# joekurina/Agilex-NTT

Measured on AMD Instinct MI355X. Metric: batched n=4096 forward NTTs/sec at 1/2/4/8 MI355X; %HBM roofline, higher is better.
Workload: dtype u64; 1 GPU; n=4096, 4-prime RNS (60-bit), batch=4096 polynomials per GPU, forward negacyclic NTT in place (BASELINE.json configs[2]); n=4096, primes=4, batch_per_gpu=4096, slabs_rotated=4, clock_ramp_steps_before_warmup=1856, parallelism=batch-sharded x1, no collective

## Files before the change

agilex-ntt_amd/csrc/agx_ntt.cpp:

```cpp
#include "../../include/agx_ntt.h"

#include <hip/hip_runtime.h>

#include <algorithm>
#include <cmath>
#include <cstdlib>
#include <cstring>
#include <memory>
#include <mutex>
#include <new>
#include <vector>

#include "host_math.hpp"
#include "operands.hpp"
#include "plan_internal.hpp"
#include "rb_registry.hpp"
#ifdef AGX_DIAG
#include "../../tools/agx_ntt_diag.h"
#endif

using namespace agx;

thread_local int g_last_hip_error = 0;

// ... 72 lines not shown

int check_modulus(uint64_t q, uint32_t n) {
    if (q < 3 || (q & 1) == 0 || q >= (1ull << 62)) return AGX_ERR_BAD_MODULUS;
    if ((q - 1) % (2ull * n)) return AGX_ERR_BAD_MODULUS;
    return AGX_OK;
}

int check_shape(uint32_t n, uint32_t num_primes) {
    if (int rc = check_size(n)) return rc;
    return num_primes == 0 || num_primes > 65535 ? AGX_ERR_BAD_ARGUMENT : AGX_OK;
}

int check_create_args(uint32_t n, uint32_t num_primes, const uint64_t* moduli, const uint64_t* tw, const uint64_t* pre, const uint64_t* itw, const uint64_t* ipre) {
    if (!moduli || !tw || !pre || (itw == nullptr) != (ipre == nullptr)) return AGX_ERR_NULL_POINTER;
    if (int rc = check_shape(n, num_primes)) return rc;
    for (uint32_t k = 0; k < num_primes; ++k)
        if (int rc = check_modulus(moduli[k], n)) return rc;
    return AGX_OK;
}

int check_plan(const agx_ntt_plan* plan) {
    if (!plan) return AGX_ERR_NULL_POINTER;
    int dev = -1;
    return hipGetDevice(&dev) == hipSuccess && dev == plan->device ? AGX_OK : AGX_ERR_BAD_ARGUMENT;
}

void free_plan(agx_ntt_plan* p) {
    if (!p) return;
    for (hipEvent_t ev : p->ticket_events)
        if (ev) (void)hipEventDestroy(ev);
    delete p;
}

static std::vector<ulonglong2> build_pass_table(const rb_entry* e, const std::vector<ulonglong2>& pairs, uint32_t num_primes, uint32_t n) {
    std::vector<ulonglong2> out;
    std::vector<uint64_t> w(n), wp(n);
    for (uint32_t k = 0; k < num_primes; ++k) {
        for (uint32_t j = 0; j < n; ++j) w[j] = pairs[(size_t)k * n + j].x, wp[j] = pairs[(size_t)k * n + j].y;
        e->build(w.data(), wp.data(), out);
    }
    return out;
}

static void resolve_routes(agx_ntt_plan* p) {
    route generic;
    generic.n = p->n, generic.log_n = p->log_n, generic.num_primes = p->num_primes;
    generic.consts = p->d_consts, generic.tw = p->d_tw, generic.itw = p->d_itw, generic.rescale = p->d_rescale;
    generic.ticket_for = &plan_ticket_for, generic.ticket_launched = &plan_ticket_launched;
    generic.ticket_ctx = p;
    auto through = [&](const pass_tables& t) {
        route r = generic;
        r.rb = t.entry, r.tw_rb = t.fwd, r.itw_rb = t.inv;
        return r;
    };
    const rb_entry* e = p->variant == AGX_VARIANT_LDS_RADIX2 ? nullptr : p->main.entry;
    const route main = e ? through(p->main) : generic;
    const bool inv = e && p->main.inv;
    plan_routes& r = p->routes;
    r.forward = main;
    const bool large = e && !p->explicit_id && p->chosen.forward_large && p->chosen.forward_large == p->companion.entry;
    r.forward_large = large ? through(p->companion) : route{};
    r.min_frames = p->chosen.min_frames;
    r.inverse = inv && e->launch_inv ? main : generic;
    r.polymul = inv && e->launch_mul ? main : generic;
    r.polymul_ntt = inv && e->launch_mulhat ? main : generic;
    r.rescale = inv && e->launch_rescale ? main : generic;
    r.extend = e && e->launch_extend ? main : generic;
    r.moddown = inv && e->launch_moddown ? main : generic;
}

static const route& forward_route(const agx_ntt_plan* p, uint64_t batch) {
    const plan_routes& r = p->routes;
// ... 48 lines not shown
        c.mu_lo = (uint64_t)mu;
        if (q >= (1ull << 58) && q <= (1ull << 60)) {
            float f = (float)(4294967296.0 / (double)q * (1.0 - 1.0 / 1048576.0));
            if ((double)f > 4294967296.0 / (double)q * (1.0 - 1.0 / 1048576.0)) f = std::nextafterf(f, 0.0f);
            uint32_t bits;
            std::memcpy(&bits, &f, sizeof(bits));
            c.est = bits;
        }
        c.est |= (uint64_t)q60c_of(q) << 32;

        c.n_inv = inv_pow2_mod(img.log_n, q);
        c.n_inv_p = shoup_quotient(c.n_inv, q);
        const uint64_t* twk = tw + (size_t)k * n;
        const uint64_t* prek = pre + (size_t)k * n;
        for (uint32_t j = 0; j < n; ++j) img.tw_pairs[(size_t)k * n + j] = make_ulonglong2(twk[j], prek[j]);
        if (itw) {
            const uint64_t* itwk = itw + (size_t)k * n;
            const uint64_t* iprek = ipre + (size_t)k * n;
            for (uint32_t j = 0; j < n; ++j) img.itw_pairs[(size_t)k * n + j] = make_ulonglong2(itwk[j], iprek[j]);
            c.w1n = mul_mod(itwk[1] % q, c.n_inv, q);
            c.w1n_p = shoup_quotient(c.w1n, q);
        }
    }
    img.rescale_legal = num_primes >= 2;
    img.rescale.assign(num_primes >= 2 ? num_primes - 1 : 0, rescale_consts{});
    for (uint32_t k = 0; k + 1 < num_primes; ++k) {
        const uint64_t q = moduli[k], q_last = moduli[num_primes - 1], h = (q_last - 1) >> 1;
        rescale_consts& rc = img.rescale[k];
        rc.q_last = q_last, rc.h = h, rc.h_mod_q = h % q;
        if (inv_mod_euclid(q_last, q, &rc.qlinv)) rc.qlinv_p = shoup_quotient(rc.qlinv, q);
        else img.rescale_legal = false;
    }
    const rb_selection& c = img.chosen;
    if (c.main) img.tables.push_back({c.main, build_pass_table(c.main, img.tw_pairs, num_primes, n), itw ? build_pass_table(c.main, img.itw_pairs, num_primes, n) : std::vector<ulonglong2>{}});
    if (c.forward_large && c.forward_large != c.main) img.tables.push_back({c.forward_large, build_pass_table(c.forward_large, img.tw_pairs, num_primes, n), {}});
}

static int upload_pass_tables(pass_tables& dst, const host_pass_tables& src) {
    dst.entry = src.entry;
    if (int rc = dst.fwd.upload(src.fwd)) return rc;
    return src.inv.empty() ? AGX_OK : dst.inv.upload(src.inv);
}

int prepare_auto_image(plan_image& img, uint32_t n, uint32_t num_primes, const uint64_t* moduli, const uint64_t* psi) {
    std::vector<uint64_t> roots(num_primes), tw((size_t)num_primes * n), pre(tw.size()), itw(tw.size()), ipre(tw.size());
    for (uint32_t k = 0; k < num_primes; ++k) {
        const uint64_t q = moduli[k];
        if (int rc = check_modulus(q, n)) return rc;
        if (!is_prime_u64(q)) return AGX_ERR_BAD_MODULUS;
        roots[k] = psi ? psi[k] : min_primitive_root_2n(q, n);
        if (!is_primitive_root_2n(roots[k], q, n)) return AGX_ERR_BAD_ROOT;
        power_tables_bitrev(q, roots[k], n, &tw[(size_t)k * n], &pre[(size_t)k * n]);
        power_tables_bitrev(q, inv_mod(roots[k], q), n, &itw[(size_t)k * n], &ipre[(size_t)k * n]);
    }
    prepare_plan_image(img, n, num_primes, moduli, roots.data(), tw.data(), pre.data(), itw.data(), ipre.data());
    return AGX_OK;
}

int instantiate_plan(agx_ntt_plan** out, const plan_image& img) {
    int ndev = 0;
    if (hipGetDeviceCount(&ndev) != hipSuccess || ndev == 0) return AGX_ERR_NO_DEVICE;
    std::unique_ptr<agx_ntt_plan, void (*)(agx_ntt_plan*)> p(new (std::nothrow) agx_ntt_plan, &free_plan);
    if (!p) return AGX_ERR_ALLOC;
    p->n = img.n, p->log_n = img.log_n, p->num_primes = img.num_primes;
    p->has_inverse = img.has_inverse, p->arith_level = img.arith_level, p->narrow_level = img.narrow_level;
    p->chosen = img.chosen;
    p->rescale_legal = img.rescale_legal;
    p->ticket_streams.reserve(kTicketSlots);
// ... 37 lines not shown
int check_frames(const agx_ntt_plan* plan, const void* base, const frame_layout& fl) {
    if (!base) return AGX_ERR_NULL_POINTER;
    if (!aligned8(base) || !batch_fits_grid(plan, fl.batch)) return AGX_ERR_BAD_ARGUMENT;
    if (fl.batch > 1 && fl.poly_stride < (int64_t)plan->n) return AGX_ERR_BAD_ARGUMENT;
    if (!layout_fits(plan->n, plan->num_primes, fl.batch, fl.prime_stride, fl.poly_stride)) return AGX_ERR_BAD_ARGUMENT;
    if (self_overlap(plan->n, plan->num_primes, fl.batch, fl.prime_stride, fl.poly_stride)) return AGX_ERR_BAD_ARGUMENT;
    return AGX_OK;
}

int check_pair(const agx_ntt_plan* plan, const void* base, const void* other, const frame_layout& fl) {
    if (!other) return AGX_ERR_NULL_POINTER;
    if (!aligned8(other)) return AGX_ERR_BAD_ARGUMENT;
    return partial_overlap(addr(base), addr(other), plan->n, plan->num_primes, fl.batch, fl.prime_stride, fl.poly_stride) ? AGX_ERR_BAD_ARGUMENT : AGX_OK;
}

static int plan_set_variant_impl(agx_ntt_plan* plan, int variant) {
    if (!plan) return AGX_ERR_NULL_POINTER;
    int config_id = -1;
    if (variant >= AGX_VARIANT_REGBLOCK_BASE) {
        config_id = variant - AGX_VARIANT_REGBLOCK_BASE;
        variant = AGX_VARIANT_REGBLOCK;
    }
    if (variant != AGX_VARIANT_AUTO && variant != AGX_VARIANT_LDS_RADIX2 && variant != AGX_VARIANT_REGBLOCK) return AGX_ERR_BAD_ARGUMENT;
    if (variant != AGX_VARIANT_LDS_RADIX2) {
        rb_selection sel = regblock_select(plan->n, config_id, plan->arith_level, plan->narrow_level);
        if (!sel.main) {
            if (variant == AGX_VARIANT_REGBLOCK) return AGX_ERR_BAD_SIZE;
            sel.main = plan->main.entry;
        }
        if (sel.main != plan->main.entry) {
            host_pass_tables host{sel.main, {}, {}};
            std::vector<ulonglong2> pairs((size_t)plan->num_primes * plan->n);
            AGX_HIP(hipMemcpy(pairs.data(), plan->d_tw, pairs.size() * sizeof(ulonglong2), hipMemcpyDeviceToHost));
            host.fwd = build_pass_table(sel.main, pairs, plan->num_primes, plan->n);
            if (plan->d_itw) {
                AGX_HIP(hipMemcpy(pairs.data(), plan->d_itw, pairs.size() * sizeof(ulonglong2), hipMemcpyDeviceToHost));
                host.inv = build_pass_table(sel.main, pairs, plan->num_primes, plan->n);
            }
            pass_tables fresh;
            if (int rc = upload_pass_tables(fresh, host)) return rc;
            AGX_HIP(hipDeviceSynchronize());
            plan->main = std::move(fresh);
        }
        plan->chosen = sel;
        plan->explicit_id = config_id >= 0;
    }
    plan->variant = variant;
    resolve_routes(plan);
    return AGX_OK;
}

}

extern "C" {

const char* agx_ntt_strerror(int status) {
    switch (status) {
        case AGX_OK: return "success";
        case AGX_ERR_NULL_POINTER: return "required pointer argument is NULL";
        case AGX_ERR_BAD_SIZE: return "n must be a power of two in [2, 32768]";
        case AGX_ERR_BAD_MODULUS: return "modulus must be an odd prime < 2^62 with q = 1 (mod 2n)";
        case AGX_ERR_BAD_ROOT: return "psi is not a primitive 2n-th root of unity mod q";
        case AGX_ERR_BAD_ARGUMENT: return "invalid argument";
        case AGX_ERR_NO_DEVICE: return "no HIP device available";
        case AGX_ERR_HIP: return "HIP runtime error (see agx_ntt_last_hip_error)";
        case AGX_ERR_ALLOC: return "allocation failed";
        case AGX_ERR_NO_INVERSE: return "plan has no inverse tables";
    }
    return "unknown status";
}
// ... 503 lines not shown
```

agilex-ntt_amd/csrc/host_math.cpp:

```cpp
#include "host_math.hpp"

namespace agx {

typedef unsigned __int128 u128;

uint64_t mul_mod(uint64_t a, uint64_t b, uint64_t q) { return (uint64_t)((u128)a * b % q); }

uint64_t pow_mod(uint64_t a, uint64_t e, uint64_t q) {
    uint64_t r = 1 % q, base = a % q;
    for (; e; e >>= 1) {
        if (e & 1) r = mul_mod(r, base, q);
        base = mul_mod(base, base, q);
    }
    return r;
}

uint64_t inv_mod(uint64_t a, uint64_t q) { return pow_mod(a, q - 2, q); }

bool is_prime_u64(uint64_t q) {
    if (q < 2) return false;
    const uint64_t wit[] = {2, 3, 5, 7, 11, 13, 17, 19, 23, 29, 31, 37};
    for (uint64_t p : wit)
        if (q % p == 0) return q == p;
    uint64_t odd = q - 1;
// ... 32 lines not shown

uint64_t min_primitive_root_2n(uint64_t q, uint32_t n) {
    const uint64_t two_n = 2ull * n;
    if (q < 3 || (q - 1) % two_n) return 0;
    const uint64_t cofactor = (q - 1) / two_n;
    uint64_t some_root = 0;
    for (uint64_t g = 2; g < q && g < 100000; ++g) {
        uint64_t r = pow_mod(g, cofactor, q);
        if (is_primitive_root_2n(r, q, n)) { some_root = r; break; }
    }
    if (!some_root) return 0;
    const uint64_t sq = mul_mod(some_root, some_root, q);
    uint64_t least = some_root, walk = some_root;
    for (uint32_t k = 1; k < n; ++k) {
        walk = mul_mod(walk, sq, q);
        if (walk < least) least = walk;
    }
    return least;
}

bool inv_mod_euclid(uint64_t a, uint64_t q, uint64_t* inv) {
    __int128 r0 = q, r1 = a % q, t0 = 0, t1 = 1;
    while (r1 != 0) {
        const __int128 k = r0 / r1, r2 = r0 - k * r1, t2 = t0 - k * t1;
        r0 = r1, r1 = r2, t0 = t1, t1 = t2;
    }
    if (r0 != 1) return false;
    *inv = (uint64_t)(t0 < 0 ? t0 + (__int128)q : t0);
    return true;
}

uint64_t shoup_quotient(uint64_t w, uint64_t q) { return (uint64_t)(((u128)w << 64) / q); }

void power_tables_bitrev(uint64_t q, uint64_t base, uint32_t n, uint64_t* tw, uint64_t* pre) {
    const int lg = log2u(n);
    std::vector<uint64_t> pw(n);
    pw[0] = 1 % q;
    for (uint32_t i = 1; i < n; ++i) pw[i] = mul_mod(pw[i - 1], base, q);
    for (uint32_t j = 0; j < n; ++j) {
        tw[j] = pw[bit_reverse(j, lg)];
        pre[j] = shoup_quotient(tw[j], q);
    }
}

bool basis_constants(const uint64_t* src, uint32_t S, const uint64_t* dst, uint32_t T, uint64_t* dinv, uint64_t* dinv_p, uint64_t* mat, uint64_t* mat_p) {
    auto d_mod = [&](uint32_t i, uint64_t m) {
        uint64_t r = 1 % m;
        for (uint32_t k = 0; k < S; ++k)
            if (k != i) r = mul_mod(r, src[k] % m, m);
        return r;
    };
    for (uint32_t i = 0; i < S; ++i) {
        if (!inv_mod_euclid(d_mod(i, src[i]), src[i], &dinv[i])) return false;
        dinv_p[i] = shoup_quotient(dinv[i], src[i]);
    }
    for (uint32_t j = 0; j < T; ++j)
        for (uint32_t i = 0; i < S; ++i) {
            mat[(std::size_t)j * S + i] = d_mod(i, dst[j]);
            mat_p[(std::size_t)j * S + i] = shoup_quotient(mat[(std::size_t)j * S + i], dst[j]);
        }
    return true;
}

bool moddown_constants(const uint64_t* src, uint32_t S, const uint64_t* dst, uint32_t T, const uint64_t* dinv, const uint64_t* n_inv, const uint64_t* w1n,
                       uint64_t* dall, uint64_t* dall_p, uint64_t* sn, uint64_t* sn_p, uint64_t* sw, uint64_t* sw_p) {
    for (uint32_t i = 0; i < S; ++i) {
// ... 18 lines not shown
```

agilex-ntt_amd/csrc/host_math.hpp:

```cpp
#pragma once
#include <cstddef>
#include <cstdint>
#include <vector>

namespace agx {

uint64_t mul_mod(uint64_t a, uint64_t b, uint64_t q);
uint64_t pow_mod(uint64_t a, uint64_t e, uint64_t q);
uint64_t inv_mod(uint64_t a, uint64_t q);
bool inv_mod_euclid(uint64_t a, uint64_t q, uint64_t* inv);
bool is_prime_u64(uint64_t q);
inline bool is_pow2(uint32_t n) { return n && !(n & (n - 1)); }
inline int log2u(uint32_t n) { int l = 0; while ((1u << l) < n) ++l; return l; }
inline uint32_t bit_reverse(uint32_t x, int bits) {
    uint32_t r = 0;
    for (int i = 0; i < bits; ++i) { r = (r << 1) | (x & 1u); x >>= 1; }
    return r;
}

std::vector<uint64_t> find_ntt_primes(uint32_t bits, uint32_t n, uint32_t count);
uint64_t min_primitive_root_2n(uint64_t q, uint32_t n);
bool is_primitive_root_2n(uint64_t psi, uint64_t q, uint32_t n);

uint64_t shoup_quotient(uint64_t w, uint64_t q);
void power_tables_bitrev(uint64_t q, uint64_t base, uint32_t n, uint64_t* tw, uint64_t* pre);

bool basis_constants(const uint64_t* src, uint32_t S, const uint64_t* dst, uint32_t T, uint64_t* dinv, uint64_t* dinv_p, uint64_t* mat, uint64_t* mat_p);

bool moddown_constants(const uint64_t* src, uint32_t S, const uint64_t* dst, uint32_t T, const uint64_t* dinv, const uint64_t* n_inv, const uint64_t* w1n,
                       uint64_t* dall, uint64_t* dall_p, uint64_t* sn, uint64_t* sn_p, uint64_t* sw, uint64_t* sw_p);

}
```

agilex-ntt_amd/csrc/modarith.hpp:

```cpp
#pragma once
#include <hip/hip_runtime.h>
#include <cstdint>

namespace agx {

typedef ulonglong2 twpair;

__device__ __forceinline__ uint64_t mul_shoup_lazy(uint64_t y, uint64_t w, uint64_t wp, uint64_t q) {
    const uint64_t c = __umul64hi(y, wp);
    return w * y - c * q;
}

__device__ __forceinline__ uint64_t csub(uint64_t v, uint64_t m) { return v >= m ? v - m : v; }

__device__ __forceinline__ uint64_t reduce_4q(uint64_t v, uint64_t q, uint64_t q2) {
    return csub(csub(v, q2), q);
}

__device__ __forceinline__ void ct_butterfly(uint64_t& x, uint64_t& y, uint64_t w, uint64_t wp,
                                             uint64_t q, uint64_t q2) {
    const uint64_t tx = csub(x, q2);
    const uint64_t qv = mul_shoup_lazy(y, w, wp, q);
    x = tx + qv;
    y = tx + q2 - qv;
// ... 43 lines not shown
}


__device__ __forceinline__ uint64_t mad64(uint32_t a, uint32_t b, uint64_t c) { return (uint64_t)a * b + c; }
__device__ __forceinline__ uint64_t mul64(uint32_t a, uint32_t b) { return (uint64_t)a * b; }

template <int TAG>
__device__ __forceinline__ uint32_t opaque_one() {
    uint32_t one;
    if constexpr (TAG == 0) asm("s_mov_b32 %0, 1" : "=s"(one));
    else asm("s_movk_i32 %0, 0x1" : "=s"(one));
    return one;
}
__device__ __forceinline__ uint64_t add64_32(uint64_t c, uint32_t a, uint32_t one) { return (uint64_t)a * one + c; }

__device__ __forceinline__ uint64_t opaque_sgpr64(uint64_t v) {
    asm("" : "+s"(v));
    return v;
}

__device__ __forceinline__ uint64_t keep64(uint64_t v) {
    asm("" : "+v"(v));
    return v;
}

struct bf_consts {
    uint64_t q;
    uint64_t nq;
    uint64_t m;
    uint64_t nm;
    uint32_t one_a, one_b;
    float est_inv;
    uint32_t c, c8;
};

__device__ __forceinline__ uint64_t csub_sign(uint64_t x, const bf_consts& k) {
    const uint64_t d = x + k.nm;
    const uint32_t neg = (uint32_t)((int32_t)(uint32_t)(d >> 32) >> 31);
    typedef uint32_t u32x2 __attribute__((ext_vector_type(2)));
    u32x2 add;
    add.x = neg & (uint32_t)k.m;
    add.y = neg & (uint32_t)(k.m >> 32);
    return d + __builtin_bit_cast(uint64_t, add);
}

template <int VAR = 0>
__device__ __forceinline__ uint64_t fold_product(uint64_t tx, uint64_t y, uint64_t w, uint64_t c, const bf_consts& k) {
    const uint32_t y0 = (uint32_t)y, y1 = (uint32_t)(y >> 32), w0 = (uint32_t)w, w1 = (uint32_t)(w >> 32);
    const uint32_t c0 = (uint32_t)c, c1 = (uint32_t)(c >> 32), nq0 = (uint32_t)k.nq, nq1 = (uint32_t)(k.nq >> 32);
    uint64_t acc = mad64(w0, y0, tx);
    acc = mad64(nq0, c0, acc);
    if constexpr (VAR == 1) {
        const uint32_t z32 = w0 * y1 + w1 * y0 + nq1 * c0 + nq0 * c1;
        typedef uint32_t u32x2v __attribute__((ext_vector_type(2)));
        u32x2v av = __builtin_bit_cast(u32x2v, acc);
        av.y += z32;
        return __builtin_bit_cast(uint64_t, av);
    }
    uint64_t z = mul64(w0, y1);
    z = mad64(w1, y0, z);
    z = mad64(nq1, c0, z);
    z = keep64(mad64(nq0, c1, z));
    typedef uint32_t u32x2 __attribute__((ext_vector_type(2)));
    u32x2 a = __builtin_bit_cast(u32x2, acc);
    a.y += (uint32_t)z;
    return __builtin_bit_cast(uint64_t, a);
// ... 176 lines not shown
        return lazy16_tailfree::valid(total);
    }
};

__device__ __forceinline__ uint64_t csub_8q_q60c(uint64_t x, const bf_consts& k) {
    typedef uint32_t u32x2 __attribute__((ext_vector_type(2)));
    u32x2 v = __builtin_bit_cast(u32x2, x);
    uint32_t s = v.y >> 31;
    asm("" : "+v"(s));
    v.y &= 0x7fffffffu;
    return mad64(s, k.c8, __builtin_bit_cast(uint64_t, v));
}

template <bool DO_CSUB>
__device__ __forceinline__ void ct_butterfly_q60c(uint64_t& x, uint64_t& y, uint64_t w, uint64_t wp, const bf_consts& k) {
    const uint32_t y0 = (uint32_t)y, y1 = (uint32_t)(y >> 32), p0 = (uint32_t)wp, p1 = (uint32_t)(wp >> 32);
    const uint64_t tx = DO_CSUB ? csub_8q_q60c(x, k) : x;
    uint64_t c = mad64(p1, y1, (uint64_t)__umulhi(y0, p1));
    c = add64_32(c, __umulhi(y1, p0), k.one_b);
    const uint64_t xn = fold_product(tx, y, w, c, k);
    y = (tx << 1) + k.m - xn;
    x = xn;
}

__device__ __forceinline__ uint64_t reduce_final_q60c(uint64_t v, const bf_consts& k, const final_consts& f, bool lazy_out) {
    typedef uint32_t u32x2 __attribute__((ext_vector_type(2)));
    u32x2 r = __builtin_bit_cast(u32x2, v);
    const uint32_t kq = r.y >> 28;
    r.y &= 0x0fffffffu;
    const uint64_t t = mad64(kq, k.c, __builtin_bit_cast(uint64_t, r));
    return lazy_out ? t : csub_select_c(t, f.nq1);
}

template <bool FAST>
__device__ __forceinline__ uint64_t mul_shoup_form(uint64_t d, uint64_t w, uint64_t wp, const bf_consts& k) {
    const uint32_t d0 = (uint32_t)d, d1 = (uint32_t)(d >> 32), p0 = (uint32_t)wp, p1 = (uint32_t)(wp >> 32);
    uint64_t c;
    if constexpr (FAST) {
        c = mad64(p1, d1, (uint64_t)__umulhi(d0, p1));
        c = add64_32(c, __umulhi(d1, p0), k.one_b);
    } else {
        const uint32_t t = __umulhi(d0, p0);
        const uint64_t m1 = add64_32(mul64(p1, d0), t, k.one_a);
        const uint64_t m2 = add64_32(mul64(p0, d1), (uint32_t)m1, k.one_b);
        c = add64_32(mul64(p1, d1), (uint32_t)(m1 >> 32), k.one_a);
        c = add64_32(c, (uint32_t)(m2 >> 32), k.one_b);
    }
    return fold_product(0, d, w, c, k);
}

template <bool FAST, bool SEL = false>
__device__ __forceinline__ void gs_butterfly_form(uint64_t& x, uint64_t& y, uint64_t w, uint64_t wp, const bf_consts& k) {
    const uint64_t s = x + y;
    const uint64_t d = x + k.m - y;
    if constexpr (FAST) x = SEL ? csub_select(s, k) : csub_sign(s, k);
    else x = csub(s, k.m);
    y = mul_shoup_form<FAST>(d, w, wp, k);
}

template <bool FAST>
__device__ __forceinline__ void gs_last_form(uint64_t& x, uint64_t& y, uint64_t ninv, uint64_t ninv_p,
                                             uint64_t w1n, uint64_t w1n_p, const bf_consts& k) {
    const uint64_t s = x + y;
    const uint64_t d = x + k.m - y;
    x = mul_shoup_form<FAST>(s, ninv, ninv_p, k);
    y = mul_shoup_form<FAST>(d, w1n, w1n_p, k);
// ... 52 lines not shown
```

agilex-ntt_amd/csrc/rb32_kernels.hpp:

```cpp
#pragma once

namespace agx {
namespace AGX_TU {

typedef uint2 tw32;
typedef unsigned long long u64x2 __attribute__((ext_vector_type(2)));

__device__ __forceinline__ tw32 load_uniform32(const tw32* p) {
    typedef const uint64_t __attribute__((address_space(4))) * const_ptr;
    const uint64_t v = *(const_ptr)(uintptr_t)p;
    return make_uint2((uint32_t)v, (uint32_t)(v >> 32));
}

__device__ __forceinline__ uint32_t csub32(uint32_t a, uint32_t m) {
    const uint32_t d = a - m;
    return d < a ? d : a;
}

template <int TIER>
struct q32_arith {
    static_assert(TIER == 1 || TIER == 2, "1: q < 2^31, 2: q < 2^30");
    uint32_t q, q2;
    __device__ __forceinline__ void init(uint64_t q64) {
        q = (uint32_t)q64;
// ... 260 lines not shown
polymul_q32(const uint64_t* __restrict__ pa, const uint64_t* __restrict__ pb, uint64_t* __restrict__ pcout, const prime_consts* __restrict__ consts,
            const twpair* __restrict__ tw_rb, const twpair* __restrict__ itw_rb, uint32_t pairs_per_prime, uint64_t frames_x,
            int64_t prime_stride, int64_t poly_stride, uint32_t flags) {
    __builtin_amdgcn_s_setprio(3);
    AGX_RB32_PROLOGUE;
    (void)wide;
    const tw32* itbl = reinterpret_cast<const tw32*>(itw_rb) + (size_t)prime * pairs_per_prime * 2;
    uint32_t xa[C], xb[C];
    {
        uint64_t va[C];
        static_for<0, C>([&](auto Rr) { constexpr int r = Rr; va[r] = __builtin_nontemporal_load(&pa[base + f.tid + (uint32_t)r * T]); });
        asm volatile("" ::: "memory");
        __builtin_amdgcn_s_setprio(0);
        static_for<0, C>([&](auto Rr) { constexpr int r = Rr; xa[r] = f.a.template enter<false>(va[r]); });
    }
    f.forward(xa, tbl, true);
    asm volatile("" ::: "memory");
    static_for<0, C>([&](auto Rr) { constexpr int r = Rr; xb[r] = f.a.template enter<false>(__builtin_nontemporal_load(&pb[base + f.tid + (uint32_t)r * T])); });
    __syncthreads();
    {
        const tw32* tbl2 = tbl;
        asm volatile("" : "+s"(tbl2));
        f.forward(xb, tbl2, true);
    }
    static_for<0, C>([&](auto Rr) { constexpr int r = Rr; xa[r] = f.a.mulmod(xa[r], xb[r], pc.mu_hi); });
    const tw32 ninv = make_uint2((uint32_t)pc.n_inv, (uint32_t)(pc.n_inv_p >> 32)), w1n = make_uint2((uint32_t)pc.w1n, (uint32_t)(pc.w1n_p >> 32));
    f.inverse(xa, itbl, ninv, w1n);
    if (live) {
        static_for<0, C>([&](auto Rr) { constexpr int r = Rr; __builtin_nontemporal_store((uint64_t)xa[r], &pcout[base + f.tid + (uint32_t)r * T]); });
    }
}

template <int L, int R>
void build_table32_t(const uint64_t* tw, const uint64_t* pre, std::vector<ulonglong2>& out) {
    using G = rb_geom<L, R>;
    static_assert(G::table_pairs % 2 == 0, "two 8-byte entries per 16-byte slot");
    std::vector<uint2> t((size_t)G::table_pairs, make_uint2(0, 0));
    for_each_table_slot<L, R>([&](size_t at, uint32_t idx) { t[at] = make_uint2((uint32_t)tw[idx], (uint32_t)(pre[idx] >> 32)); });
    const size_t start = out.size();
    out.resize(start + (size_t)G::table_pairs / 2);
    std::memcpy(out.data() + start, t.data(), t.size() * sizeof(uint2));
}

template <int L, int R, int PPB, int TIER, int MINW>
struct q32_shape {
    static constexpr int log_n = L, r = R, fpb = PPB, threads = rb_geom<L, R>::T * PPB, min_waves = MINW, arith = 1, narrow = TIER;
    static constexpr uint32_t table_pairs = rb_geom<L, R>::table_pairs / 2;
    static constexpr size_t lds = (size_t)((1u << L) + (1u << (L - 5))) * 4 * PPB;
    static constexpr auto build = &build_table32_t<L, R>;
    static constexpr bool flags_everywhere = true;
    static uint32_t flags(const void* a, const void* b, const void* c, const frame_layout& fl) {
        const bool aligned = (((uintptr_t)a | (uintptr_t)b | (uintptr_t)c) & 15u) == 0 && ((fl.prime_stride | fl.poly_stride) & 1) == 0;
        return (fl.lazy_out ? 1u : 0u) | (aligned ? 2u : 0u);
    }
};

template <int L, int R, int PPB, int TIER, int MINW>
constexpr rb_entry make_entry_q32(int id) {
    return make_entry3<q32_shape<L, R, PPB, TIER, MINW>, &fwd_q32<L, R, PPB, TIER, MINW>, &inv_q32<L, R, PPB, TIER, MINW>, &polymul_q32<L, R, PPB, TIER, MINW>>(id);
}

}
}
```

agilex-ntt_amd/csrc/rb_frame.hpp:

```cpp
#pragma once
#include "rb_registry.hpp"
#include "modarith.hpp"

#include <algorithm>
#include <cstdlib>
#include <type_traits>
#include <utility>

#ifndef AGX_POLYMUL_MAXW
#define AGX_POLYMUL_MAXW 5
#endif
#ifndef AGX_TU
#error "define AGX_TU (a per-translation-unit namespace name) before including rb_frame.hpp / rb_kernels.hpp"
#endif

namespace agx {
namespace AGX_TU {



template <int B, int E, typename F>
__device__ __host__ __forceinline__ void static_for(F&& f) {
    if constexpr (B < E) {
        f(std::integral_constant<int, B>{});
// ... 60 lines not shown
    return {r0, r0 | (1 << rb), b >> rb};
}

struct no_op {
    __device__ __forceinline__ void operator()() const {}
};
template <int C, class WR, class RD, class SYNC, class MID = no_op>
__device__ __forceinline__ void split_words_out(const uint64_t (&x)[C], uint32_t* w, uint32_t (&lo)[C], WR&& wr, RD&& rd, SYNC&& sync, MID&& mid = MID{}) {
    static_for<0, C>([&](auto r) { w[wr(r)] = (uint32_t)x[r]; });
    mid();
    sync();
    static_for<0, C>([&](auto r) { lo[r] = w[rd(r)]; });
    sync();
    static_for<0, C>([&](auto r) { w[wr(r)] = (uint32_t)(x[r] >> 32); });
    sync();
}

constexpr int kOptPad = 1;
constexpr int kOptSelect = 2;
constexpr int kOptLazy16 = 16;
constexpr int kOptTwAhead = 32;
constexpr int kOptTrace = 64;
constexpr int kOptPrio = 128;
constexpr int kOptPrioBarrier = 512;
constexpr int kOptScalarBase = 1024;
constexpr int kOptLazyInv = 2048;
constexpr int kOptTwAheadInv = 4096;
constexpr int kOptNtLoad = 131072, kOptNtStore = 262144;
constexpr int kOptEstReduce = 524288;
constexpr int kOptSplitWord = 1048576;
constexpr int kOptStreamTw = 1 << 25;
constexpr int kOptPinBf = 1 << 26;
constexpr int kOptQ60c = 1 << 27;
constexpr int kOptStreamCh1 = 1 << 29;

#ifdef AGX_DIAG
__device__ uint64_t* g_trace_buf = nullptr;
__device__ uint64_t g_trace_waves = 0;
#endif

template <int L, int R, bool FAST, int OPT = 0>
struct rb2_frame {
    using G = rb2_geom<L, R>;
    static constexpr int C = G::C, T = G::T, NP = G::NP;
    static constexpr bool FAST_ARITH = FAST, SEL = (OPT & kOptSelect) != 0, LAZY16 = FAST && (OPT & kOptLazy16) != 0;
    static_assert((OPT & kOptPad) != 0, "every kernel uses the padded image");
    static constexpr bool TWA = (OPT & kOptTwAhead) != 0 && R >= 3;
    static constexpr bool TRACE = (OPT & kOptTrace) != 0;
    static constexpr bool PRIO = (OPT & kOptPrio) != 0;
    static constexpr bool PRIO_BARRIER = PRIO && (OPT & kOptPrioBarrier) != 0, SCALAR_BASE = (OPT & kOptScalarBase) != 0;
    static constexpr bool LAZY_INV = LAZY16 && (OPT & kOptLazyInv) != 0;
    static constexpr bool NT_LOAD = (OPT & kOptNtLoad) != 0, NT_STORE = (OPT & kOptNtStore) != 0;
    static constexpr bool TWA_INV = (OPT & kOptTwAheadInv) != 0 && R == 3;
    static constexpr bool EST = LAZY16 && SEL && (OPT & kOptEstReduce) != 0;
    static constexpr bool Q60C = EST && (OPT & kOptQ60c) != 0;
    static constexpr bool SPLIT = (OPT & kOptSplitWord) != 0;
    static constexpr bool STREAM_TW = (OPT & kOptStreamTw) != 0, PIN_BF = (OPT & kOptPinBf) != 0, STREAM_CH1 = (OPT & kOptStreamCh1) != 0;
    static_assert(!EST || lazy16_tailfree::valid(L), "tail-free schedule must keep every stage within 16q");
    static_assert(!Q60C || q60c_tailfree::valid(L), "sign-bit subtracts must keep every stage within 16q + 8c");
    mutable uint64_t ts[12];
    uint64_t trace_wave = ~0ull;
    bool trace_wait_stores = true;
    template <int I>
    __device__ __forceinline__ void stamp(uint64_t& anchor) const {
        if constexpr (TRACE) {
            uint64_t t;
            asm volatile("s_memtime %0\n\ts_waitcnt lgkmcnt(0)" : "=s"(t), "+v"(anchor) : : "memory");
            ts[I] = t;
        }
    }
    __device__ __forceinline__ void trace_flush() const {
#ifndef AGX_DIAG
        static_assert(!TRACE, "kOptTrace kernels belong to the diagnostics library (AGX_DIAG): the product library has no trace buffer");
#else
        if constexpr (TRACE) {
            const uint64_t wave = ((uint64_t)blockIdx.y * gridDim.x + blockIdx.x) * (blockDim.x >> 6) + (threadIdx.x >> 6);
            if ((threadIdx.x & 63u) == 0 && g_trace_buf != nullptr && wave < g_trace_waves) {
                uint64_t* dst = g_trace_buf + wave * 16;
#pragma unroll
                for (int i = 0; i < 12; ++i) dst[i] = ts[i];
                dst[12] = __builtin_amdgcn_s_getreg((31 << 11) | 4);
                dst[13] = __builtin_amdgcn_s_getreg((31 << 11) | 20);
            }
        }
#endif
    }
    static constexpr bool lane_full_pass(int p) { return p >= 0 && p < NP && G::rlo(p) < 6 && G::hi(p) - G::rlo(p) + 1 == R; }
    static constexpr int PADS = SPLIT ? 5 : 4;
    static constexpr uint32_t slab_elems = (1u << L) + (L >= PADS ? (1u << (L >= PADS ? L - PADS : 0)) : 0u);
    static constexpr uint32_t image_bytes = slab_elems * (SPLIT ? 4u : 8u);
    static __device__ __forceinline__ constexpr uint32_t img(uint32_t e) { return e + (e >> PADS); }
    uint32_t tid;
    bool lazy_out = false;
    uint64_t* slab;
    bf_consts k;
    final_consts fc;

    __device__ __forceinline__ void init_consts(uint64_t q, uint64_t est = 0) {
        k.est_inv = __uint_as_float((uint32_t)est);
        k.q = q;
        k.nq = 0 - q;
        k.m = FAST ? (q << 2) : (q << 1);
        k.nm = opaque_sgpr64(0 - k.m);
        k.one_a = opaque_one<0>();
        k.one_b = opaque_one<1>();
        fc.q2 = q << 1;
        fc.nq2 = opaque_sgpr64(0 - fc.q2);
        fc.q1 = q;
        fc.nq1 = opaque_sgpr64(0 - fc.q1);
        fc.q8 = q << 3;
        fc.nq8 = opaque_sgpr64(0 - fc.q8);
        if constexpr (Q60C) {
            k.c = (uint32_t)(est >> 32);
            k.c8 = k.c << 3;
        }
    }

    template <int stage>
    __device__ __forceinline__ void butterfly(uint64_t& a, uint64_t& b, const twpair& w) const {
        if constexpr (Q60C) ct_butterfly_q60c<lazy16_tailfree::subtracts(stage, L)>(a, b, w.x, w.y, k);
        else if constexpr (EST) ct_butterfly_lazy16<SEL, lazy16_tailfree::subtracts(stage, L), false>(a, b, w.x, w.y, k, fc);
        else if constexpr (LAZY16) ct_butterfly_lazy16<SEL, lazy16_schedule::subtracts(stage), stage == L - 1>(a, b, w.x, w.y, k, fc);
        else if constexpr (FAST) ct_butterfly_fast<SEL>(a, b, w.x, w.y, k);
        else ct_butterfly_exact(a, b, w.x, w.y, k);
    }

    template <int stage, int MODE>
    __device__ __forceinline__ void forward_step(uint64_t& a, uint64_t& b, const twpair& w) const {
        butterfly<stage>(a, b, w);
        if constexpr (stage == L - 1) {
            a = final_reduce<MODE>(a);
            b = final_reduce<MODE>(b);
        }
    }
    template <int gap, int BND, class TW>
    __device__ __forceinline__ void inverse_step(uint64_t& a, uint64_t& b, const prime_consts& pc, TW&& tw) const {
        if constexpr (gap == L - 1) {
            if constexpr (LAZY_INV) gs_last_lazy16<BND, SEL>(a, b, pc.n_inv, pc.n_inv_p, pc.w1n, pc.w1n_p, k, fc);
            else gs_last_form<FAST>(a, b, pc.n_inv, pc.n_inv_p, pc.w1n, pc.w1n_p, k);
            a = reduce_final_inv<FAST, SEL>(a, k, fc);
            b = reduce_final_inv<FAST, SEL>(b, k, fc);
        } else {
            const twpair w = tw();
            if constexpr (LAZY_INV) gs_butterfly_lazy16<BND, SEL>(a, b, w.x, w.y, k, fc);
            else gs_butterfly_form<FAST, SEL>(a, b, w.x, w.y, k);
        }
    }
    static constexpr int inv_b0(int p) { return p == NP - 1 ? 4 : 8; }
    template <int p>
    __device__ __forceinline__ void inverse_pass_cleanup(uint64_t (&x)[C]) const {
        if constexpr (LAZY_INV && p > 0) {
            static_for<0, C>([&](auto Rr) {
                constexpr int r = Rr;
// ... 423 lines not shown
```

agilex-ntt_amd/csrc/rb_kernels.hpp:

```cpp
#pragma once
#include "rb_frame.hpp"

#ifndef AGX_MULHAT_MAXW
#define AGX_MULHAT_MAXW 6
#endif
namespace agx {
namespace AGX_TU {

template <int L, int R, int ARITH>
using frame_of = rb2_frame<L, R, (ARITH & 1) == 1, (ARITH >> 1)>;

#define AGX_RB2_PROLOGUE                                                                          \
    using F = frame_of<L, R, ARITH>;                                                              \
    constexpr int C = F::C, T = F::T;                                                             \
    static_assert(T >= 64, "one frame must span whole waves");                                    \
    F f;                                                                                          \
    f.tid = threadIdx.x & (T - 1);                                                                \
    const uint32_t slot = threadIdx.x / T;                                                        \
    uint64_t fx = (uint64_t)blockIdx.x * PPB + slot;                                              \
    const bool live = fx < frames_x;                                                              \
    if (!live) fx = frames_x - 1;                          \
    const uint32_t prime = blockIdx.y;                                                            \
    f.init_consts(consts[prime].q, consts[prime].est);                                            \
    f.slab = reinterpret_cast<uint64_t*>(agx_dyn_lds) + (size_t)slot * F::slab_elems;             \
    const int64_t base = (int64_t)prime * prime_stride + (int64_t)fx * poly_stride

template <int L, int R, int PPB, int ARITH, int MINW>
__global__ void __launch_bounds__((1 << (L - R)) * PPB, MINW)
fwd_rb2(const uint64_t* __restrict__ in, uint64_t* __restrict__ out,
        const prime_consts* __restrict__ consts, const twpair* __restrict__ tw_rb,
        uint32_t pairs_per_prime, uint64_t frames_x,
        int64_t prime_stride, int64_t poly_stride, uint32_t lazy_out) {
    uint64_t t_entry = 0;
    if constexpr (frame_of<L, R, ARITH>::TRACE) asm volatile("s_memtime %0\n\ts_waitcnt lgkmcnt(0)" : "=s"(t_entry) : : "memory");
// ... 465 lines not shown
            uint64_t v = w[EARLY ? g : (g & 1)][i / 2][i & 1];
            if constexpr (!F::LAZY16) v = reduce_4q(v, q, q2);
            asm volatile("" : "+v"(acc[r]));
            acc[r] = rescale_finish<F::LAZY16>(v, acc[r], d.x, d.y, q);
            asm volatile("" : "+v"(acc[r]));
        });
        __builtin_amdgcn_sched_barrier(0);
    });
    f.store_last_layout(acc, out, base, live);
}


template <int L, int R, class F>
void for_each_table_slot(F&& f) {
    using G = rb2_geom<L, R>;
    for (int p = 0; p < G::NP; ++p) {
        const int rlo = G::rlo(p), hi = G::hi(p), H = G::H(p);
        for (int j = 1; j < G::C; ++j) {
            int k = 0;
            while ((2 << k) <= j) ++k;
            const int o = j - (1 << k), rb_bit = R - 1 - k, b = rlo + rb_bit;
            if (b > hi) continue;
            const uint32_t m_local = 1u << (L - 1 - b);
            for (int h = 0; h < H; ++h) {
                const uint32_t idx = m_local + ((uint32_t)h << k) + (uint32_t)o;
                const size_t at = G::uniform_pass(p) ? (size_t)h * G::C + j : (size_t)j * H + h;
                f((size_t)G::table_off(p) + at, idx);
            }
        }
    }
}

template <int L, int R>
void build_table_t(const uint64_t* tw, const uint64_t* pre, std::vector<ulonglong2>& out) {
    const size_t start = out.size();
    out.resize(start + (size_t)rb_geom<L, R>::table_pairs, make_ulonglong2(0, 0));
    for_each_table_slot<L, R>([&](size_t at, uint32_t idx) { out[start + at] = make_ulonglong2(tw[idx], pre[idx]); });
}

template <class F>
constexpr int rb2_arith_level() { return F::Q60C ? 3 : F::LAZY16 ? 2 : F::FAST_ARITH ? 1 : 0; }

struct lazy_flag {
    static constexpr bool flags_everywhere = false;
    static uint32_t flags(const void*, const void*, const void*, const frame_layout& fl) { return fl.lazy_out ? 1u : 0u; }
};

template <int L, int R, int PPB, int ARITH, int MINW>
struct rb2_shape : lazy_flag {
    static constexpr int log_n = L, r = R, fpb = PPB, threads = rb_geom<L, R>::T * PPB, min_waves = MINW, arith = rb2_arith_level<frame_of<L, R, ARITH>>(), narrow = 0;
    static constexpr uint32_t table_pairs = rb_geom<L, R>::table_pairs;
    static constexpr size_t lds = (size_t)frame_of<L, R, ARITH>::image_bytes * PPB;
    static constexpr auto build = &build_table_t<L, R>;
};

template <size_t BYTES, auto... K>
hipError_t allow_lds() {
    hipError_t e = hipSuccess;
    ((e = e != hipSuccess ? e : hipFuncSetAttribute(reinterpret_cast<const void*>(K), hipFuncAttributeMaxDynamicSharedMemorySize, (int)BYTES)), ...);
    return e;
}

template <class S, class K, class... A>
hipError_t launch_frames(K kernel, const plan_view& pv, const frame_layout& fl, hipStream_t s, A... args) {
    const dim3 grid((unsigned)((fl.batch + S::fpb - 1) / S::fpb), pv.num_primes);
    hipLaunchKernelGGL(kernel, grid, dim3(S::threads), S::lds, s, args...);
    return hipGetLastError();
}

template <class S, auto K>
hipError_t launch_fwd_t(const plan_view& pv, const uint64_t* in, uint64_t* out, const frame_layout& fl, hipStream_t s) {
    return launch_frames<S>(K, pv, fl, s, in, out, pv.consts, pv.tw_rb, pv.rb->table_pairs, fl.batch, fl.prime_stride, fl.poly_stride,
                            S::flags(in, out, nullptr, fl));
}

template <class S, auto K>
hipError_t launch_inv_t(const plan_view& pv, const uint64_t* in, const uint64_t* in2, uint64_t* out, const frame_layout& fl, hipStream_t s) {
    if constexpr (S::flags_everywhere)
        return launch_frames<S>(K, pv, fl, s, in, in2, out, pv.consts, pv.itw_rb, pv.rb->table_pairs, fl.batch, fl.prime_stride, fl.poly_stride,
                                S::flags(in, in2, out, fl));
    else
        return launch_frames<S>(K, pv, fl, s, in, in2, out, pv.consts, pv.itw_rb, pv.rb->table_pairs, fl.batch, fl.prime_stride, fl.poly_stride);
}

template <class S, auto K>
hipError_t launch_mul_t(const plan_view& pv, const uint64_t* a, const uint64_t* b, uint64_t* c, const frame_layout& fl, hipStream_t s) {
// ... 172 lines not shown
```

agilex-ntt_amd/csrc/rb_registry.hpp:

```cpp
#pragma once
#include "ntt_kernels.hpp"

namespace agx {

struct rb_entry {
    int id, log_n, r, ppb;
    int min_waves;
    uint32_t table_pairs;
    size_t lds_bytes;
    void (*build)(const uint64_t* tw, const uint64_t* pre, std::vector<ulonglong2>& out);
    hipError_t (*launch)(const plan_view&, const uint64_t*, uint64_t*, const frame_layout&, hipStream_t);
    hipError_t (*init)();
    int arith;
    hipError_t (*launch_inv)(const plan_view&, const uint64_t*, const uint64_t*, uint64_t*, const frame_layout&, hipStream_t);
    hipError_t (*launch_mul)(const plan_view&, const uint64_t*, const uint64_t*, uint64_t*, const frame_layout&, hipStream_t);
    int fwd_companion = 0;
    uint32_t fwd_companion_min_frames = 0;
    int narrow = 0;
    hipError_t (*launch_mulhat)(const plan_view&, const uint64_t*, const uint64_t*, uint64_t*, const frame_layout&, int64_t bhat_prime_stride,
                                int64_t bhat_poly_stride, hipStream_t) = nullptr;
    hipError_t (*launch_rescale)(const plan_view&, const uint64_t* x, const uint64_t* t, uint64_t* out, const frame_layout&, bool round, hipStream_t) = nullptr;
    hipError_t (*launch_extend)(const plan_view&, const basis_view&, const uint64_t* x, uint64_t* out, const frame_layout&, hipStream_t) = nullptr;
    hipError_t (*launch_moddown)(const plan_view&, const basis_view&, const uint64_t* xq, const uint64_t* y, uint64_t* out, const frame_layout&, hipStream_t) = nullptr;
};

inline plan_view prime_range(plan_view v, uint32_t lo, uint32_t hi) {
    v.consts += lo;
    v.tw += (size_t)lo * v.n;
    if (v.itw) v.itw += (size_t)lo * v.n;
    if (v.tw_rb) v.tw_rb += (size_t)lo * v.rb->table_pairs;
    if (v.itw_rb) v.itw_rb += (size_t)lo * v.rb->table_pairs;
    if (v.rescale) v.rescale += lo;
    v.num_primes = hi - lo;
    return v;
}

struct rb_span {
    const rb_entry* first;
    size_t count;
};

rb_span rb_entries_n4096();
rb_span rb_entries_s1024();
// ... 16 lines not shown
```

agilex-ntt_amd/csrc/reg_s4096.hip:

```cpp
#define AGX_TU tu_s4096
#include "rb_kernels.hpp"
#include "rb_stream_opts.hpp"

namespace agx {
namespace AGX_TU {
const rb_entry kEntries[] = {
    make_entry_single_fwd<12, 5, kLazy | (kOptPrio << 1), 4>(159),
    make_entry_single_fwd<12, 5, kLazy | ((kOptPrio | kOptQ60c) << 1), 4>(165),
#ifdef AGX_DIAG
    make_entry_single<12, 5, kLazy | (kOptPrio << 1), 4>(147),
    make_entry_single<12, 4, kLazy | (kOptStreamCh1 << 1), 8>(161),
#endif
};
}

rb_span rb_entries_s4096() { return rb_span{AGX_TU::kEntries, sizeof(AGX_TU::kEntries) / sizeof(AGX_TU::kEntries[0])}; }

}
```

Measured before the change: 59.95 million NTT/s.

## Use folded two-twiddle butterfly for q = 2^60 - c NTT kernel

Adds a new Cooley-Tukey butterfly for 60-bit primes of the form 2^60 - c that replaces the Shoup quotient with a second precomputed twiddle (w*2^32 mod q), packed in a 29-bit split. The product is then folded through multiply-adds by 2^29 and 2c, with no high-word quotient multiply. The host table builder now receives the modulus so it can produce the packed twiddle pairs, and entry 165 is switched to the new form while the old one is kept under diagnostics. This is meant to cut the integer multiply count per butterfly. It relies on static bounds that hold only for c below 2^28, and it changes the lazy-reduction schedule.

```diff
diff --git a/agilex-ntt_amd/csrc/agx_ntt.cpp b/agilex-ntt_amd/csrc/agx_ntt.cpp
--- a/agilex-ntt_amd/csrc/agx_ntt.cpp
+++ b/agilex-ntt_amd/csrc/agx_ntt.cpp
@@ -128,12 +128,13 @@
     delete p;
 }
 
-static std::vector<ulonglong2> build_pass_table(const rb_entry* e, const std::vector<ulonglong2>& pairs, uint32_t num_primes, uint32_t n) {
+static std::vector<ulonglong2> build_pass_table(const rb_entry* e, const std::vector<ulonglong2>& pairs, const std::vector<uint64_t>& moduli, uint32_t n) {
+    const uint32_t num_primes = (uint32_t)moduli.size();
     std::vector<ulonglong2> out;
     std::vector<uint64_t> w(n), wp(n);
     for (uint32_t k = 0; k < num_primes; ++k) {
         for (uint32_t j = 0; j < n; ++j) w[j] = pairs[(size_t)k * n + j].x, wp[j] = pairs[(size_t)k * n + j].y;
-        e->build(w.data(), wp.data(), out);
+        e->build(w.data(), wp.data(), moduli[k], out);
     }
     return out;
 }
@@ -248,8 +249,8 @@
         else img.rescale_legal = false;
     }
     const rb_selection& c = img.chosen;
-    if (c.main) img.tables.push_back({c.main, build_pass_table(c.main, img.tw_pairs, num_primes, n), itw ? build_pass_table(c.main, img.itw_pairs, num_primes, n) : std::vector<ulonglong2>{}});
-    if (c.forward_large && c.forward_large != c.main) img.tables.push_back({c.forward_large, build_pass_table(c.forward_large, img.tw_pairs, num_primes, n), {}});
+    if (c.main) img.tables.push_back({c.main, build_pass_table(c.main, img.tw_pairs, img.moduli, n), itw ? build_pass_table(c.main, img.itw_pairs, img.moduli, n) : std::vector<ulonglong2>{}});
+    if (c.forward_large && c.forward_large != c.main) img.tables.push_back({c.forward_large, build_pass_table(c.forward_large, img.tw_pairs, img.moduli, n), {}});
 }
 
 static int upload_pass_tables(pass_tables& dst, const host_pass_tables& src) {
@@ -353,10 +354,10 @@
             host_pass_tables host{sel.main, {}, {}};
             std::vector<ulonglong2> pairs((size_t)plan->num_primes * plan->n);
             AGX_HIP(hipMemcpy(pairs.data(), plan->d_tw, pairs.size() * sizeof(ulonglong2), hipMemcpyDeviceToHost));
-            host.fwd = build_pass_table(sel.main, pairs, plan->num_primes, plan->n);
+            host.fwd = build_pass_table(sel.main, pairs, plan->moduli, plan->n);
             if (plan->d_itw) {
                 AGX_HIP(hipMemcpy(pairs.data(), plan->d_itw, pairs.size() * sizeof(ulonglong2), hipMemcpyDeviceToHost));
-                host.inv = build_pass_table(sel.main, pairs, plan->num_primes, plan->n);
+                host.inv = build_pass_table(sel.main, pairs, plan->moduli, plan->n);
             }
             pass_tables fresh;
             if (int rc = upload_pass_tables(fresh, host)) return rc;
diff --git a/agilex-ntt_amd/csrc/host_math.cpp b/agilex-ntt_amd/csrc/host_math.cpp
--- a/agilex-ntt_amd/csrc/host_math.cpp
+++ b/agilex-ntt_amd/csrc/host_math.cpp
@@ -88,6 +88,11 @@
 
 uint64_t shoup_quotient(uint64_t w, uint64_t q) { return (uint64_t)(((u128)w << 64) / q); }
 
+fold_twiddle fold_twiddle_pack(uint64_t w, uint64_t q) {
+    const uint64_t low29 = (1ull << 29) - 1, wc = mul_mod(w, 1ull << 32, q);
+    return {(w & low29) | (w >> 29) << 32, (wc & low29) | (wc >> 29) << 32};
+}
+
 void power_tables_bitrev(uint64_t q, uint64_t base, uint32_t n, uint64_t* tw, uint64_t* pre) {
     const int lg = log2u(n);
     std::vector<uint64_t> pw(n);
diff --git a/agilex-ntt_amd/csrc/host_math.hpp b/agilex-ntt_amd/csrc/host_math.hpp
--- a/agilex-ntt_amd/csrc/host_math.hpp
+++ b/agilex-ntt_amd/csrc/host_math.hpp
@@ -25,6 +25,11 @@
 uint64_t shoup_quotient(uint64_t w, uint64_t q);
 void power_tables_bitrev(uint64_t q, uint64_t base, uint32_t n, uint64_t* tw, uint64_t* pre);
 
+struct fold_twiddle {
+    uint64_t w_packed, wc_packed;
+};
+fold_twiddle fold_twiddle_pack(uint64_t w, uint64_t q);
+
 bool basis_constants(const uint64_t* src, uint32_t S, const uint64_t* dst, uint32_t T, uint64_t* dinv, uint64_t* dinv_p, uint64_t* mat, uint64_t* mat_p);
 
 bool moddown_constants(const uint64_t* src, uint32_t S, const uint64_t* dst, uint32_t T, const uint64_t* dinv, const uint64_t* n_inv, const uint64_t* w1n,
diff --git a/agilex-ntt_amd/csrc/modarith.hpp b/agilex-ntt_amd/csrc/modarith.hpp
--- a/agilex-ntt_amd/csrc/modarith.hpp
+++ b/agilex-ntt_amd/csrc/modarith.hpp
@@ -99,6 +99,8 @@
     uint32_t one_a, one_b;
     float est_inv;
     uint32_t c, c8;
+    uint32_t c2, p29;
+    uint64_t m8;
 };
 
 __device__ __forceinline__ uint64_t csub_sign(uint64_t x, const bf_consts& k) {
@@ -341,6 +343,42 @@
     return lazy_out ? t : csub_select_c(t, f.nq1);
 }
 
+struct q60c_fold_bounds {
+    typedef unsigned __int128 u128;
+    static constexpr u128 two64 = (u128)1 << 64, w32 = 0xffffffffull;
+    static constexpr u128 c_max = (1ull << 28) - 1, q_min = (1ull << 60) - (uint64_t)c_max, q_max = (1ull << 60) - 1;
+    static constexpr u128 wh_max = (uint64_t)q_max >> 29, wl_max = (1ull << 29) - 1;
+    static constexpr u128 hi_max = 2 * w32 * wh_max;
+    static constexpr u128 lo_max = 2 * w32 * wl_max;
+    static constexpr u128 Q_max = lo_max + w32 * ((u128)1 << 29) + w32 * 2 * c_max;
+    static constexpr u128 tx_max = ((u128)1 << 63) + 8 * c_max - 1, tx_max_c1 = ((u128)1 << 63) + 8 - 1;
+    static_assert(wh_max < ((u128)1 << 31), "the high half of a twiddle fits 31 bits");
+    static_assert(hi_max < two64, "hi fits 64 bits");
+    static_assert(tx_max + Q_max < two64, "x' = tx + Q does not wrap (every partial sum of the chain is below this one)");
+    static_assert(Q_max <= 8 * q_min, "y' = tx + 8q - Q is not negative");
+    static_assert(tx_max + 8 * q_min < two64 && tx_max_c1 + 8 * q_max < two64, "y' <= tx + 8q = 2^64 - 1 for every c");
+};
+
+__device__ __forceinline__ uint32_t opaque_two29() {
+    uint32_t v;
+    asm("s_mov_b32 %0, 0x20000000" : "=s"(v));
+    return v;
+}
+
+template <bool DO_CSUB>
+__device__ __forceinline__ void ct_butterfly_q60c_fold(uint64_t& x, uint64_t& y, uint64_t w, uint64_t wC, const bf_consts& k) {
+    const uint32_t y0 = (uint32_t)y, y1 = (uint32_t)(y >> 32);
+    const uint32_t wl = (uint32_t)w, wh = (uint32_t)(w >> 32), wCl = (uint32_t)wC, wCh = (uint32_t)(wC >> 32);
+    const uint64_t tx = DO_CSUB ? csub_8q_q60c(x, k) : x;
+    const uint64_t hi = mad64(y1, wCh, mul64(y0, wh));
+    uint64_t xn = keep64(mad64(y0, wl, tx));
+    xn = mad64(y1, wCl, xn);
+    xn = mad64((uint32_t)hi, k.p29, xn);
+    xn = mad64((uint32_t)(hi >> 32), k.c2, xn);
+    y = (tx << 1) + k.m8 - xn;
+    x = xn;
+}
+
 template <bool FAST>
 __device__ __forceinline__ uint64_t mul_shoup_form(uint64_t d, uint64_t w, uint64_t wp, const bf_consts& k) {
     const uint32_t d0 = (uint32_t)d, d1 = (uint32_t)(d >> 32), p0 = (uint32_t)wp, p1 = (uint32_t)(wp >> 32);
diff --git a/agilex-ntt_amd/csrc/rb32_kernels.hpp b/agilex-ntt_amd/csrc/rb32_kernels.hpp
--- a/agilex-ntt_amd/csrc/rb32_kernels.hpp
+++ b/agilex-ntt_amd/csrc/rb32_kernels.hpp
@@ -316,7 +316,7 @@
 }
 
 template <int L, int R>
-void build_table32_t(const uint64_t* tw, const uint64_t* pre, std::vector<ulonglong2>& out) {
+void build_table32_t(const uint64_t* tw, const uint64_t* pre, uint64_t, std::vector<ulonglong2>& out) {
     using G = rb_geom<L, R>;
     static_assert(G::table_pairs % 2 == 0, "two 8-byte entries per 16-byte slot");
     std::vector<uint2> t((size_t)G::table_pairs, make_uint2(0, 0));
diff --git a/agilex-ntt_amd/csrc/rb_frame.hpp b/agilex-ntt_amd/csrc/rb_frame.hpp
--- a/agilex-ntt_amd/csrc/rb_frame.hpp
+++ b/agilex-ntt_amd/csrc/rb_frame.hpp
@@ -116,6 +116,7 @@
 constexpr int kOptStreamTw = 1 << 25;
 constexpr int kOptPinBf = 1 << 26;
 constexpr int kOptQ60c = 1 << 27;
+constexpr int kOptQ60cFold = 1 << 28;
 constexpr int kOptStreamCh1 = 1 << 29;
 
 #ifdef AGX_DIAG
@@ -138,6 +139,8 @@
     static constexpr bool TWA_INV = (OPT & kOptTwAheadInv) != 0 && R == 3;
     static constexpr bool EST = LAZY16 && SEL && (OPT & kOptEstReduce) != 0;
     static constexpr bool Q60C = EST && (OPT & kOptQ60c) != 0;
+    static constexpr bool Q60C_FOLD = Q60C && (OPT & kOptQ60cFold) != 0;
+    static_assert((OPT & kOptQ60cFold) == 0 || Q60C, "the two-twiddle butterfly is a form of the q = 2^60 - c kernels");
     static constexpr bool SPLIT = (OPT & kOptSplitWord) != 0;
     static constexpr bool STREAM_TW = (OPT & kOptStreamTw) != 0, PIN_BF = (OPT & kOptPinBf) != 0, STREAM_CH1 = (OPT & kOptStreamCh1) != 0;
     static_assert(!EST || lazy16_tailfree::valid(L), "tail-free schedule must keep every stage within 16q");
@@ -198,11 +201,17 @@
             k.c = (uint32_t)(est >> 32);
             k.c8 = k.c << 3;
         }
+        if constexpr (Q60C_FOLD) {
+            k.c2 = k.c << 1;
+            k.p29 = opaque_two29();
+            k.m8 = q << 3;
+        }
     }
 
     template <int stage>
     __device__ __forceinline__ void butterfly(uint64_t& a, uint64_t& b, const twpair& w) const {
-        if constexpr (Q60C) ct_butterfly_q60c<lazy16_tailfree::subtracts(stage, L)>(a, b, w.x, w.y, k);
+        if constexpr (Q60C_FOLD) ct_butterfly_q60c_fold<(stage >= 1)>(a, b, w.x, w.y, k);
+        else if constexpr (Q60C) ct_butterfly_q60c<lazy16_tailfree::subtracts(stage, L)>(a, b, w.x, w.y, k);
         else if constexpr (EST) ct_butterfly_lazy16<SEL, lazy16_tailfree::subtracts(stage, L), false>(a, b, w.x, w.y, k, fc);
         else if constexpr (LAZY16) ct_butterfly_lazy16<SEL, lazy16_schedule::subtracts(stage), stage == L - 1>(a, b, w.x, w.y, k, fc);
         else if constexpr (FAST) ct_butterfly_fast<SEL>(a, b, w.x, w.y, k);
diff --git a/agilex-ntt_amd/csrc/rb_kernels.hpp b/agilex-ntt_amd/csrc/rb_kernels.hpp
--- a/agilex-ntt_amd/csrc/rb_kernels.hpp
+++ b/agilex-ntt_amd/csrc/rb_kernels.hpp
@@ -1,5 +1,6 @@
 #pragma once
 #include "rb_frame.hpp"
+#include "host_math.hpp"
 
 #ifndef AGX_MULHAT_MAXW
 #define AGX_MULHAT_MAXW 6
@@ -531,10 +532,19 @@
 }
 
 template <int L, int R>
-void build_table_t(const uint64_t* tw, const uint64_t* pre, std::vector<ulonglong2>& out) {
+void build_table_t(const uint64_t* tw, const uint64_t* pre, uint64_t, std::vector<ulonglong2>& out) {
     const size_t start = out.size();
     out.resize(start + (size_t)rb_geom<L, R>::table_pairs, make_ulonglong2(0, 0));
     for_each_table_slot<L, R>([&](size_t at, uint32_t idx) { out[start + at] = make_ulonglong2(tw[idx], pre[idx]); });
+}
+template <int L, int R>
+void build_table_fold_t(const uint64_t* tw, const uint64_t*, uint64_t q, std::vector<ulonglong2>& out) {
+    const size_t start = out.size();
+    out.resize(start + (size_t)rb_geom<L, R>::table_pairs, make_ulonglong2(0, 0));
+    for_each_table_slot<L, R>([&](size_t at, uint32_t idx) {
+        const fold_twiddle f = fold_twiddle_pack(tw[idx], q);
+        out[start + at] = make_ulonglong2(f.w_packed, f.wc_packed);
+    });
 }
 
 template <class F>
@@ -550,7 +560,7 @@
     static constexpr int log_n = L, r = R, fpb = PPB, threads = rb_geom<L, R>::T * PPB, min_waves = MINW, arith = rb2_arith_level<frame_of<L, R, ARITH>>(), narrow = 0;
     static constexpr uint32_t table_pairs = rb_geom<L, R>::table_pairs;
     static constexpr size_t lds = (size_t)frame_of<L, R, ARITH>::image_bytes * PPB;
-    static constexpr auto build = &build_table_t<L, R>;
+    static constexpr auto build = frame_of<L, R, ARITH>::Q60C_FOLD ? &build_table_fold_t<L, R> : &build_table_t<L, R>;
 };
 
 template <size_t BYTES, auto... K>
diff --git a/agilex-ntt_amd/csrc/rb_registry.hpp b/agilex-ntt_amd/csrc/rb_registry.hpp
--- a/agilex-ntt_amd/csrc/rb_registry.hpp
+++ b/agilex-ntt_amd/csrc/rb_registry.hpp
@@ -8,7 +8,7 @@
     int min_waves;
     uint32_t table_pairs;
     size_t lds_bytes;
-    void (*build)(const uint64_t* tw, const uint64_t* pre, std::vector<ulonglong2>& out);
+    void (*build)(const uint64_t* tw, const uint64_t* pre, uint64_t q, std::vector<ulonglong2>& out);
     hipError_t (*launch)(const plan_view&, const uint64_t*, uint64_t*, const frame_layout&, hipStream_t);
     hipError_t (*init)();
     int arith;
diff --git a/agilex-ntt_amd/csrc/reg_s4096.hip b/agilex-ntt_amd/csrc/reg_s4096.hip
--- a/agilex-ntt_amd/csrc/reg_s4096.hip
+++ b/agilex-ntt_amd/csrc/reg_s4096.hip
@@ -6,8 +6,9 @@
 namespace AGX_TU {
 const rb_entry kEntries[] = {
     make_entry_single_fwd<12, 5, kLazy | (kOptPrio << 1), 4>(159),
-    make_entry_single_fwd<12, 5, kLazy | ((kOptPrio | kOptQ60c) << 1), 4>(165),
+    make_entry_single_fwd<12, 5, kLazy | ((kOptPrio | kOptQ60c | kOptQ60cFold) << 1), 4>(165),
 #ifdef AGX_DIAG
+    make_entry_single_fwd<12, 5, kLazy | ((kOptPrio | kOptQ60c) << 1), 4>(167),
     make_entry_single<12, 5, kLazy | (kOptPrio << 1), 4>(147),
     make_entry_single<12, 4, kLazy | (kOptStreamCh1 << 1), 8>(161),
 #endif
```

Measured after the change: 67.64 million NTT/s (median of 6 runs). 12.8% higher.
